# halixness/distributed-3d-diffusion-pytorch

Measured on AMD Instinct MI355X. Metric: train imgs/sec (whole node), SRN cars 64x64 bs128, higher is better.
Workload: dtype bf16; 1 GPU; model=XUNet ch128 ch_mult(1,2,2,4) 136.7M params (3DiM, reference xunet.py), global_batch=128, seq_len=4096, image_size=64, per_gpu_batch=128, micro_batch=128, hip_graph=False, parallelism=dp1, dist_backend=none, tuned_gemms=True, backend=hip

## Files before the change

distributed_3d_diffusion_pytorch_amd/ops/csrc/conv.hip:

```cpp
#include "common.h"
#include <stdlib.h>

#include <algorithm>

D3D_API int d3d_colsum(const float* in, long R, int Cc, float* part, float* out, float* out_odd, int accumulate,
                       hipStream_t st);

typedef __attribute__((ext_vector_type(4))) short s16x4;
typedef __attribute__((ext_vector_type(8))) short s16x8;
typedef __attribute__((address_space(3))) s16x4 lds_s16x4;

namespace {

template <int TAPS, bool TRANS>
__global__ void __launch_bounds__(256, 2)
conv_glds_k(const bf16* __restrict__ I, const bf16* __restrict__ Wp, const float* __restrict__ bias,
            const float* __restrict__ row_bias, const bf16* __restrict__ res, bf16* __restrict__ O,
            const bf16* __restrict__ zero16, int Nimg, int IH, int IW, int IC, int ICp, int OH, int OW, int OC,
            int ldo, int stride, float scale, int res_nmod, float* __restrict__ part, int korder) {
  constexpr int BM = 128, BN = 128, BKk = 64;
  constexpr int WM = 64, WN = 64, TM = 4, TN = 4;
  constexpr int STAGE = (BM + BN) * BKk;
  __shared__ __attribute__((aligned(16))) bf16 smem[2 * STAGE];
  typedef __attribute__((address_space(3))) void lds_void;
// ... 1799 lines not shown
struct WSegs {
  int n;
  int row0[kMaxSegs + 1];
  float* w[kMaxSegs];
  float* b[kMaxSegs];
};

__device__ __forceinline__ int seg_of(const WSegs& sg, int co) {
  int s = 0;
  while (s + 1 < sg.n && co >= sg.row0[s + 1]) ++s;
  return s;
}

__global__ void wgrad_reduce_seg_k(const float* __restrict__ ws, int OC, int IC, int splits, int accumulate,
                                   int taps, const float* __restrict__ bws, int brows, WSegs sg) {
  long total = (long)OC * IC * taps;
  if (bws) {
    for (long c = blockIdx.x * (long)blockDim.x + threadIdx.x; c < OC; c += (long)gridDim.x * blockDim.x) {
      float s = 0.f;
      for (int k = 0; k < brows; ++k) s += bws[(long)k * OC + c];
      int g = seg_of(sg, (int)c);
      float* d = sg.b[g];
      if (d) {
        d += c - sg.row0[g];
        *d = accumulate ? *d + s : s;
      }
    }
  }
  for (long t = blockIdx.x * (long)blockDim.x + threadIdx.x; t < total; t += (long)gridDim.x * blockDim.x) {
    int ci = (int)(t % IC);
    long r = t / IC;
    int tap = (int)(r % taps);
    int co = (int)(r / taps);
    float s0 = 0.f, s1 = 0.f, s2 = 0.f, s3 = 0.f;
    int k = 0;
    for (; k + 4 <= splits; k += 4) {
      s0 += ws[(long)k * total + t];
      s1 += ws[(long)(k + 1) * total + t];
      s2 += ws[(long)(k + 2) * total + t];
      s3 += ws[(long)(k + 3) * total + t];
    }
    for (; k < splits; ++k) s0 += ws[(long)k * total + t];
    float s = (s0 + s1) + (s2 + s3);
    int g = seg_of(sg, co);
    float* d = sg.w[g] + (((long)(co - sg.row0[g]) * IC + ci) * taps + tap);
    *d = accumulate ? *d + s : s;
  }
}

template <int SL>
__global__ void __launch_bounds__(256) wgrad_reduce2_k(const float* __restrict__ ws, int OC, int IC, int taps,
                                                       int splits, int accumulate, const float* __restrict__ bws,
                                                       int brows, float* __restrict__ dW, float* __restrict__ db,
                                                       WSegs sg, int nblk_w, float scale) {
  constexpr int COLS = 256 / SL;
  __shared__ f32x4 red[SL][COLS];
  const int col = threadIdx.x % COLS, sl = threadIdx.x / COLS;
  const bool is_bias = blockIdx.x >= nblk_w;
  const long total = is_bias ? (long)OC : (long)OC * IC * taps;
  const float* src = is_bias ? bws : ws;
  const int nrows = is_bias ? brows : splits;
  const long base = (long)(is_bias ? blockIdx.x - nblk_w : blockIdx.x) * (COLS * 4) + col * 4;
  f32x4 a = {0.f, 0.f, 0.f, 0.f};
  if (base < total) {
    if (base + 3 < total) {
      f32x4 b2 = {0.f, 0.f, 0.f, 0.f};
      int k = sl;
      for (; k + SL < nrows; k += 2 * SL) {
        a += *reinterpret_cast<const f32x4*>(src + (long)k * total + base);
        b2 += *reinterpret_cast<const f32x4*>(src + (long)(k + SL) * total + base);
      }
      if (k < nrows) a += *reinterpret_cast<const f32x4*>(src + (long)k * total + base);
      a += b2;
    } else {
      for (int k = sl; k < nrows; k += SL)
        for (int e = 0; e < 4 && base + e < total; ++e) a[e] += src[(long)k * total + base + e];
    }
  }
  red[sl][col] = a;
  __syncthreads();
  if (sl == 0) {
    f32x4 t = red[0][col];
#pragma unroll
    for (int k = 1; k < SL; ++k) t += red[k][col];
    t *= scale;
    for (int e = 0; e < 4; ++e) {
      const long o = base + e;
      if (o >= total) break;
      float* d;
      if (is_bias) {
        const int c = (int)o;
        if (sg.n > 0) {
          const int g = seg_of(sg, c);
          d = sg.b[g] ? sg.b[g] + (c - sg.row0[g]) : nullptr;
        } else {
          d = db ? db + c : nullptr;
        }
      } else {
        const int ci = (int)(o % IC);
        const long r = o / IC;
        const int tap = (int)(r % taps);
        const int co = (int)(r / taps);
        if (sg.n > 0) {
          const int g = seg_of(sg, co);
          d = sg.w[g] + (((long)(co - sg.row0[g]) * IC + ci) * taps + tap);
        } else {
          d = dW + (((long)co * IC + ci) * taps + tap);
        }
      }
      if (d) *d = accumulate ? *d + t[e] : t[e];
    }
// ... 433 lines not shown
  if (g_conv_impl != CONV_HALO || IC % HALO_CH || OC % 128 || (W != 32 && W != 64) || in_bytes >= (1L << 31) ||
      w_bytes >= (1L << 31) || IC > 512)
    return 0;
  auto nblk = [&](int bn) { return H % (bn / W) ? 0L : (long)N * (H / (bn / W)) * (OC / 128); };
  if ((W != 32 || g_halo_w32) && nblk(512) >= 256) return 0;
  if (W == 32 && g_halo_w32s && nblk(256) >= 256) {
    *tile = 256;
    return 1;
  }
  return 0;
}

D3D_API int d3d_conv3_gn_ok(int N, int H, int W, int IC, int OC) {
  int t = 0;
  return conv3_gn_shape(N, H, W, IC, OC, &t);
}

D3D_API int d3d_conv3_gn(const void* I, const void* Wp, const float* bias, void* O, int N, int H, int W, int IC,
                         int ICp, int OC, float* gnp, int gn_groups, int* gn_done, const float* gab, hipStream_t st) {
  int tile = 0;
  if (gn_done) *gn_done = 0;
  if (!conv3_gn_shape(N, H, W, IC, OC, &tile) || ICp != (IC + 63) / 64 * 64) return -2;
  if (gnp) {
    const int Cg = gn_groups > 0 && OC % gn_groups == 0 ? OC / gn_groups : 0;
    if (!((Cg == 4 || Cg == 8 || Cg == 16 || Cg == 32) && (H * W) % 64 == 0)) gnp = nullptr;
  }
  const long in_bytes = (long)N * H * W * IC * 2, w_bytes = (long)((OC + 127) / 128 * 128) * 9 * ICp * 2;
  dim3 gh((unsigned)(N * (H / (tile / W))), (unsigned)(OC / 128), 1);
  hipLaunchKernelGGL((conv_halo_k<32, false, 256, false, false, true>), gh, dim3(512), 0, st, (const bf16*)I,
                     (const bf16*)Wp, bias, (const float*)nullptr, (const bf16*)nullptr, (bf16*)O, (int)in_bytes,
                     (int)w_bytes, N, H, IC, ICp, OC, 1.f, 0, gnp, gn_groups, (bf16*)nullptr, gab);
  if (gn_done && gnp) *gn_done = 1;
  return (int)hipGetLastError();
}

static void launch_reduce2(const float* ws, int OC, int IC, int taps, int splits, int accumulate, const float* bws,
                           int brows, float* dW, float* db, WSegs sg, bool want_bias, hipStream_t st,
                           float scale = 1.f) {
  if (taps == 9 && sg.n == 0) {
    const long base = (long)OC * ((IC + 63) / 64);
    const int tg = base >= 1024 ? 9 : (base * 3 >= 1024 ? 3 : 1);
    const int nblk_w = (int)(base * (9 / tg));
    const int nblk_b = want_bias ? (OC + 63) / 64 : 0;
#define R9(TGv) hipLaunchKernelGGL(wgrad_reduce9_k<TGv>, dim3(nblk_w + nblk_b), dim3(256), 0, st, ws, OC, IC, splits, \
                                  accumulate, bws, brows, dW, db, nblk_w, scale)
    if (tg == 9) R9(9); else if (tg == 3) R9(3); else R9(1);
#undef R9
    return;
  }
  int SL = 1;
  while (SL < splits && SL < 16) SL <<= 1;
  const long total = (long)OC * IC * taps;
  const int per = 4 * (256 / SL);
  const int nblk_w = (int)((total + per - 1) / per);
  const int nblk_b = want_bias ? (OC + per - 1) / per : 0;
  dim3 grid(nblk_w + nblk_b);
#define RL(S) hipLaunchKernelGGL(wgrad_reduce2_k<S>, grid, dim3(256), 0, st, ws, OC, IC, taps, splits, accumulate, \
                                 bws, brows, dW, db, sg, nblk_w, scale)
  switch (SL) {
    case 1: RL(1); break;
    case 2: RL(2); break;
    case 4: RL(4); break;
    case 8: RL(8); break;
    default: RL(16); break;
  }
#undef RL
}

static void launch_wgrad(const void* dY, const void* I, float* ws, int N, int IH, int IW, int IC, int OH, int OW,
                         int OC, int stride, int pps, int ncb, float* bws, int lw, int lh, int taps, dim3 grid,
                         hipStream_t st, const void* I2 = nullptr, int C1 = 0) {
  constexpr int BM = 128, BN = 128;
  const long in_elems = (long)N * IH * IW * IC;
  const bool wide_long = taps == 1 && (long)OC * IC >= (4L << 20) && pps > 16384;
  const bool fast = stride == 1 && lw >= 0 && IH == OH && IW == OW && IC % 128 == 0;
  if (g_wgrad_impl >= WGRAD_BUFL && !wide_long && (fast || in_elems * 2 < (1L << 31) - (1L << 20)) &&
      (long)pps * OC * 2 < (1L << 31)) {
    constexpr int PK = 32;
#define WB(TP, F)                                                                                                \
  hipLaunchKernelGGL((conv_wgrad_bufl_k<TP, PK, F>), grid, dim3(256), 0, st, (const bf16*)dY, (const bf16*)I, ws,   \
                     (long)N * IH * IW, N, IH, IW, IC, OH, OW, OC, stride, pps, ncb, bws, lw, lh, (const bf16*)I2, C1)
    if (taps == 9 && IC == 64 && !fast && I2 == nullptr) {
      dim3 gp(5, grid.y, grid.z);
      hipLaunchKernelGGL((conv_wgrad_bufl_k<9, PK, false, true>), gp, dim3(256), 0, st, (const bf16*)dY,
                         (const bf16*)I, ws, (long)N * IH * IW, N, IH, IW, IC, OH, OW, OC, stride, pps, 1, bws, lw, lh,
                         (const bf16*)nullptr, 0);
    } else if (taps == 9) {
      if (fast) WB(9, true); else WB(9, false);
    } else {
      if (fast) WB(1, true); else WB(1, false);
    }
#undef WB
    return;
  }
  if (taps == 9)
    hipLaunchKernelGGL((conv_wgrad_k<BM, BN, 9>), grid, dim3(256), 0, st, (const bf16*)dY, (const bf16*)I, ws, N, IH,
                       IW, IC, OH, OW, OC, stride, pps, ncb, bws, lw, lh);
  else
    hipLaunchKernelGGL((conv_wgrad_k<BM, BN, 1>), grid, dim3(256), 0, st, (const bf16*)dY, (const bf16*)I, ws, N, IH,
                       IW, IC, OH, OW, OC, stride, pps, ncb, bws, lw, lh);
}

D3D_API int d3d_conv_wgrad_plan2(int N, int OH, int OW, int OC, int IC, int taps, int* splits, int* pix_per_split) {
  constexpr int BM = 128, BN = 128;
  long P = (long)N * OH * OW;
  int tiles = (taps == 9 && IC == 64 ? 5 : taps * ((IC + BN - 1) / BN)) * ((OC + BM - 1) / BM);
  static const long target = 1024;
  static const bool ceil_ = false;
  long want = ceil_ ? (target + tiles - 1) / tiles : target / tiles;
  long maxs = (P + 255) / 256;
  if (want > maxs) want = maxs;
// ... 180 lines not shown
```

distributed_3d_diffusion_pytorch_amd/ops/csrc/reduce.hip:

```cpp
#include "common.h"

__global__ void __launch_bounds__(256) colsum_part_k(const float* __restrict__ in, long R, int Cc, int rows_per,
                                                     float* __restrict__ part) {
  __shared__ float red[8][33];
  const int c = blockIdx.x * 32 + (threadIdx.x & 31);
  const int rl = threadIdx.x >> 5;
  const long r0 = (long)blockIdx.y * rows_per;
  long r1 = r0 + rows_per;
  if (r1 > R) r1 = R;
  float s = 0.f;
  if (c < Cc)
    for (long r = r0 + rl; r < r1; r += 8) s += in[r * Cc + c];
  red[rl][threadIdx.x & 31] = s;
  __syncthreads();
  if (rl == 0 && c < Cc) {
#pragma unroll
    for (int k = 1; k < 8; ++k) s += red[k][threadIdx.x & 31];
    part[(long)blockIdx.y * Cc + c] = s;
  }
}

namespace {
__global__ void colsum_final_k(const float* __restrict__ part, int RS, int Cc, float* __restrict__ out,
                               float* __restrict__ out_odd, int accumulate) {
  int c = blockIdx.x * blockDim.x + threadIdx.x;
  if (c >= Cc) return;
  float s = 0.f;
  for (int k = 0; k < RS; ++k) s += part[(long)k * Cc + c];
  float* dst = out;
  int idx = c;
  if (out_odd) {
    dst = (c & 1) ? out_odd : out;
    idx = c >> 1;
  }
  dst[idx] = accumulate ? dst[idx] + s : s;
}
}

D3D_API int d3d_colsum(const float* in, long R, int Cc, float* part, float* out, float* out_odd, int accumulate,
                       hipStream_t st) {
  int RS = (int)((R + 63) / 64);
  if (RS > 64) RS = 64;
  if (RS < 1) RS = 1;
  int rows_per = (int)((R + RS - 1) / RS);
  hipLaunchKernelGGL(colsum_part_k, dim3((Cc + 31) / 32, RS), dim3(256), 0, st, in, R, Cc, rows_per, part);
  hipLaunchKernelGGL(colsum_final_k, dim3((Cc + 255) / 256), dim3(256), 0, st, part, RS, Cc, out, out_odd,
                     accumulate);
  return (int)hipGetLastError();
}

struct ColJob {
  const float* in;
  float* out0;
  float* out1;
  int R, Cc, acc, blk0;
};
constexpr int kMaxColJobs = 16;
struct ColJobs {
  ColJob j[kMaxColJobs];
  int n;
};

namespace {
__global__ void __launch_bounds__(256) colsum_jobs_k(ColJobs t) {
  int k = 0;
#pragma unroll 1
  while (k + 1 < t.n && (int)blockIdx.x >= t.j[k + 1].blk0) ++k;
  const ColJob& J = t.j[k];
  const int c = ((int)blockIdx.x - J.blk0) * 256 + (int)threadIdx.x;
  if (c >= J.Cc) return;
  const float* p = J.in + c;
  const long ld = J.Cc;
  float s = 0.f;
  int r = 0;
  for (; r + 8 <= J.R; r += 8) {
    float v[8];
#pragma unroll
    for (int u = 0; u < 8; ++u) v[u] = p[(long)(r + u) * ld];
#pragma unroll
    for (int u = 0; u < 8; ++u) s += v[u];
  }
  for (; r < J.R; ++r) s += p[(long)r * ld];
  float* dst = (c & 1) ? J.out1 : J.out0;
  const int idx = c >> 1;
  dst[idx] = J.acc ? dst[idx] + s : s;
}
}

D3D_API int d3d_colsum_jobs(const ColJob* jobs, int njobs, hipStream_t st) {
  if (njobs < 1 || njobs > kMaxColJobs) return (int)hipErrorInvalidValue;
  ColJobs t{};
  t.n = njobs;
  int blk = 0;
  for (int i = 0; i < njobs; ++i) {
    t.j[i] = jobs[i];
    if (t.j[i].Cc % 2 || t.j[i].R < 1 || !t.j[i].in || !t.j[i].out0 || !t.j[i].out1) return (int)hipErrorInvalidValue;
    t.j[i].blk0 = blk;
    blk += (t.j[i].Cc + 255) / 256;
  }
  hipLaunchKernelGGL(colsum_jobs_k, dim3(blk), dim3(256), 0, st, t);
  return (int)hipGetLastError();
}
```

distributed_3d_diffusion_pytorch_amd/ops/csrc/small_gemm.hip:

```cpp
#include "common.h"

namespace {
constexpr int SG_T = 64, SG_K = 16;
}

__global__ void __launch_bounds__(256) sgemm_strided_k(const float* __restrict__ A, const float* __restrict__ B,
                                                       float* __restrict__ C, int M, int N, int K, long sab, long sam,
                                                       long sak, long sbb, long sbk, long sbn, long scb, long scm,
                                                       long scn, float alpha, float beta) {
  __shared__ float As[SG_K][SG_T + 1];
  __shared__ float Bs[SG_K][SG_T + 1];
  const int b = blockIdx.z;
  const int m0 = blockIdx.y * SG_T, n0 = blockIdx.x * SG_T;
  const int tx = threadIdx.x & 15, ty = threadIdx.x >> 4;
  const float* a = A + (long)b * sab;
  const float* bb = B + (long)b * sbb;
  float acc[4][4] = {};
  for (int k0 = 0; k0 < K; k0 += SG_K) {
    for (int e = threadIdx.x; e < SG_K * SG_T; e += 256) {
      const int kk = e / SG_T, mm = e % SG_T;
      const int gm = m0 + mm, gk = k0 + kk;
      As[kk][mm] = (gm < M && gk < K) ? a[gm * sam + gk * sak] : 0.f;
      const int gn = n0 + mm;
      Bs[kk][mm] = (gn < N && gk < K) ? bb[gk * sbk + gn * sbn] : 0.f;
    }
    __syncthreads();
#pragma unroll
    for (int kk = 0; kk < SG_K; ++kk) {
      float av[4], bv[4];
#pragma unroll
      for (int i = 0; i < 4; ++i) av[i] = As[kk][ty + 16 * i];
#pragma unroll
      for (int j = 0; j < 4; ++j) bv[j] = Bs[kk][tx + 16 * j];
#pragma unroll
      for (int i = 0; i < 4; ++i)
#pragma unroll
        for (int j = 0; j < 4; ++j) acc[i][j] = __builtin_fmaf(av[i], bv[j], acc[i][j]);
    }
    __syncthreads();
  }
  float* c = C + (long)b * scb;
#pragma unroll
  for (int i = 0; i < 4; ++i) {
    const int gm = m0 + ty + 16 * i;
    if (gm >= M) continue;
#pragma unroll
    for (int j = 0; j < 4; ++j) {
      const int gn = n0 + tx + 16 * j;
      if (gn >= N) continue;
      float* d = c + gm * scm + gn * scn;
      *d = beta == 0.f ? alpha * acc[i][j] : alpha * acc[i][j] + beta * *d;
    }
  }
}

D3D_API int d3d_sgemm_strided(const float* A, const float* B, float* C, int M, int N, int K, int batch, long sab,
                              long sam, long sak, long sbb, long sbk, long sbn, long scb, long scm, long scn,
                              float alpha, float beta, hipStream_t st) {
  if (M <= 0 || N <= 0 || K <= 0 || batch <= 0 || batch > 65535) return -1;
  dim3 grid(cdiv(N, SG_T), cdiv(M, SG_T), batch);
  if (grid.y > 65535) return -1;
  hipLaunchKernelGGL(sgemm_strided_k, grid, dim3(256), 0, st, A, B, C, M, N, K, sab, sam, sak, sbb, sbk, sbn, scb,
                     scm, scn, alpha, beta);
  return (int)hipGetLastError();
}

struct SgJob {
  const float* A;
  const float* B;
  float* C;
  bf16* Cb;
  bf16* CbT;
  const float* u;
  const float* v;
  long sam, sak, sbk, sbn, scm, scn;
  int M, N, K, ldb, ldbt, tile0;
  float alpha, beta;
};
static_assert(sizeof(SgJob) == 136, "SgJob must match hip_impl._SgJob");

constexpr int SJ_K = 32;

__global__ void __launch_bounds__(256) sgemm_jobs_k(const SgJob* __restrict__ jobs, int njobs) {
  __shared__ float As[SJ_K][SG_T + 1];
  __shared__ float Bs[SJ_K][SG_T + 1];
  int j = 0;
  while (j + 1 < njobs && (int)blockIdx.x >= jobs[j + 1].tile0) ++j;
  const SgJob& J = jobs[j];
  const int t = blockIdx.x - J.tile0;
  const int ntn = (J.N + SG_T - 1) / SG_T;
  const int m0 = (t / ntn) * SG_T, n0 = (t % ntn) * SG_T;
  const int tx = threadIdx.x & 15, ty = threadIdx.x >> 4;
  float acc[4][4] = {};
  const bool a_k = J.sak == 1, b_k = J.sbk == 1;
  if (J.A) {
    for (int k0 = 0; k0 < J.K; k0 += SJ_K) {
      for (int e = threadIdx.x; e < SJ_K * SG_T; e += 256) {
        int kk = e / SG_T, mm = e % SG_T;
        if (a_k) { kk = e % SJ_K; mm = e / SJ_K; }
        const int gm = m0 + mm, gk = k0 + kk;
        As[kk][mm] = (gm < J.M && gk < J.K) ? J.A[gm * J.sam + gk * J.sak] : 0.f;
        int kb = e / SG_T, nn = e % SG_T;
        if (b_k) { kb = e % SJ_K; nn = e / SJ_K; }
        const int gn = n0 + nn, gkb = k0 + kb;
        Bs[kb][nn] = (gn < J.N && gkb < J.K) ? J.B[gkb * J.sbk + gn * J.sbn] : 0.f;
      }
      __syncthreads();
#pragma unroll 8
      for (int kk = 0; kk < SJ_K; ++kk) {
        float av[4], bv[4];
#pragma unroll
        for (int i = 0; i < 4; ++i) av[i] = As[kk][ty + 16 * i];
#pragma unroll
        for (int q = 0; q < 4; ++q) bv[q] = Bs[kk][tx + 16 * q];
#pragma unroll
        for (int i = 0; i < 4; ++i)
#pragma unroll
          for (int q = 0; q < 4; ++q) acc[i][q] = __builtin_fmaf(av[i], bv[q], acc[i][q]);
      }
      __syncthreads();
    }
  }
#pragma unroll
  for (int i = 0; i < 4; ++i) {
    const int gm = m0 + ty + 16 * i;
    if (gm >= J.M) continue;
    const float um = J.u ? J.u[gm] : 0.f;
#pragma unroll
    for (int q = 0; q < 4; ++q) {
      const int gn = n0 + tx + 16 * q;
      if (gn >= J.N) continue;
      float r = J.alpha * acc[i][q];
      if (J.C && J.beta != 0.f) r += J.beta * J.C[gm * J.scm + gn * J.scn];
      if (J.u) r += um * (J.v ? J.v[gn] : 1.f);
      if (J.C) J.C[gm * J.scm + gn * J.scn] = r;
      if (J.Cb) J.Cb[(long)gm * J.ldb + gn] = (bf16)r;
      if (J.CbT) J.CbT[(long)gn * J.ldbt + gm] = (bf16)r;
    }
  }
}

D3D_API int d3d_sgemm_jobs(const void* jobs, int njobs, int tiles, hipStream_t st) {
  if (njobs <= 0 || tiles <= 0) return -1;
  hipLaunchKernelGGL(sgemm_jobs_k, dim3((unsigned)tiles), dim3(256), 0, st, (const SgJob*)jobs, njobs);
  return (int)hipGetLastError();
}
```

distributed_3d_diffusion_pytorch_amd/ops/csrc/wgrad_group.hip:

```cpp
#include "common.h"

#include <algorithm>

namespace {

typedef __attribute__((ext_vector_type(4))) short gs16x4;
typedef __attribute__((ext_vector_type(8))) short gs16x8;
typedef __attribute__((address_space(3))) gs16x4 glds_s16x4;

__device__ __forceinline__ gs16x4 gw_tr(const bf16* p) {
  return __builtin_amdgcn_ds_read_tr16_b64_v4i16((glds_s16x4*)(p));
}

__device__ __forceinline__ gs16x4 gw_tr_asm(const bf16* p) {
  gs16x4 v;
  const unsigned a = (unsigned)(uintptr_t)(const __attribute__((address_space(3))) void*)p;
  asm volatile("ds_read_b64_tr_b16 %0, %1" : "=v"(v) : "v"(a) : "memory");
  return v;
}
template <int TM, int TN>
__device__ __forceinline__ void gw_tr_wait(bf16x8 (&a)[TM], bf16x8 (&b)[TN]) {
  asm volatile("s_waitcnt lgkmcnt(0)" ::: "memory");
#pragma unroll
  for (int i = 0; i < TM; ++i) asm volatile("" : "+v"(a[i]));
#pragma unroll
  for (int j = 0; j < TN; ++j) asm volatile("" : "+v"(b[j]));
}
__device__ __forceinline__ float gw_dot2(unsigned a, unsigned b, float c) {
  return __builtin_amdgcn_fdot2_f32_bf16(__builtin_bit_cast(bf16x2, a), __builtin_bit_cast(bf16x2, b), c, false);
}

__device__ __forceinline__ __amdgpu_buffer_rsrc_t gw_rsrc(const void* p, long bytes) {
  const unsigned long long a = (unsigned long long)p;
  const unsigned lo = __builtin_amdgcn_readfirstlane((unsigned)a);
  const unsigned hi = __builtin_amdgcn_readfirstlane((unsigned)(a >> 32));
  const int n = __builtin_amdgcn_readfirstlane((int)(bytes > 0 ? (bytes < 0x7fffffffL ? bytes : 0x7fffffffL) : 0));
  return __builtin_amdgcn_make_buffer_rsrc((void*)(((unsigned long long)hi << 32) | lo), (short)0, n, 0x00020000);
}

constexpr int GW_MAX = 16;
constexpr int GW_BM = 128, GW_BN = 128;

struct GwJob {
  const bf16* dy;
  const bf16* x;
  const bf16* x2;
  float* dw;
  float* db;
  float* slab;
  float* bslab;
  long P;
  int OC, IC, C1, taps, H, W, lw, lh, ncb, nmb, splits, pps, blk0, acc;
  float scale;
  int pad_;
};
struct GwTable {
  int n, pad_;
  GwJob j[GW_MAX];
};

struct GrJob {
  const float* slab;
  const float* bslab;
  float* dw;
  float* db;
  int OC, IC, taps, splits, blk0, nblk_w, acc;
  float scale;
  int flat, pad_;
};
struct GrTable {
  int n, pad_;
  GrJob j[GW_MAX];
};

template <int PK>
__device__ __forceinline__ void gw_issue(bf16* sA, bf16* sB, const bf16* __restrict__ dY, const bf16* __restrict__ I,
                                         long in_elems, long p0, long p_end, int OC, int IC, int OH, int OW, int kh,
                                         int kw, int dpix, int lw, int wave, const int* trow, const unsigned* aoff,
                                         const unsigned* boff, const bool* bok, bool on = true) {
  typedef __attribute__((address_space(3))) void lds_void;
  constexpr int PPW = PK / 16;
  const __amdgpu_buffer_rsrc_t rA = gw_rsrc(dY + p0 * OC, on ? (p_end - p0) * OC * 2 : 0);
#pragma unroll
  for (int i = 0; i < PPW; ++i)
    __builtin_amdgcn_raw_ptr_buffer_load_lds(rA, (lds_void*)(sA + (wave * PPW + i) * 4 * GW_BM), 16, aoff[i], 0, 0,
                                             0);
  const long pb = p0 + dpix;
  const __amdgpu_buffer_rsrc_t rB = gw_rsrc(I + pb * IC, on ? (in_elems - pb * IC) * 2 : 0);
  const int wedge = kw == 0 ? 0 : OW - 1, hedge = kh == 0 ? 0 : OH - 1;
#pragma unroll
  for (int i = 0; i < PPW; ++i) {
    const int pp = (int)p0 + trow[i];
    bool bad = !bok[i];
    if (kw != 1) bad |= (pp & (OW - 1)) == wedge;
    if (kh != 1) bad |= ((pp >> lw) & (OH - 1)) == hedge;
    __builtin_amdgcn_raw_ptr_buffer_load_lds(rB, (lds_void*)(sB + (wave * PPW + i) * 4 * GW_BN), 16,
                                             bad ? 0x80000000u : boff[i], 0, 0, 0);
  }
}

}

template <int PK, int NS>
__global__ void __launch_bounds__(256, 2) wgrad_grp_k(GwTable tab) {
  constexpr int BM = GW_BM, BN = GW_BN;
  constexpr int PER = 2 * (PK / 16);
  constexpr int WM = 64, WN = 64, TM = 4, TN = 4;
  constexpr int STAGE = PK * (BM + BN);
  constexpr int PPW = PK / 16;
  __shared__ __attribute__((aligned(16))) bf16 smem[NS * STAGE];
  const int tid = threadIdx.x, lane = tid & 63;
  const int wave = __builtin_amdgcn_readfirstlane(tid >> 6);
  const int wm = wave >> 1, wn = wave & 1;
  int R;
  {
    const int T = gridDim.x, L = blockIdx.x;
    const int q = T / 8, r = T % 8, xcd = L % 8;
    R = (xcd < r ? xcd * (q + 1) : r * (q + 1) + (xcd - r) * q) + L / 8;
  }
  int k = 0;
  while (k + 1 < tab.n && R >= tab.j[k + 1].blk0) ++k;
// ... 373 lines not shown

  const int fr = lane & 15, fq = lane >> 4;
  const int cig = ci0g + 16 * wn + fr;
  const int cw = m0 + 64 * wm;
  if (bias_wave) {
#pragma unroll
    for (int i = 0; i < 4; ++i) {
      bsum[i] += __shfl_xor(bsum[i], 16);
      bsum[i] += __shfl_xor(bsum[i], 32);
    }
  }
  if (splits == 1) {
    const float sc = J.scale;
    const int acc_in = J.acc;
    if (bias_wave && fq == 0) {
#pragma unroll
      for (int i = 0; i < 4; ++i) {
        float* d = J.db + cw + i * 16 + fr;
        const float v = bsum[i] * sc;
        *d = acc_in ? *d + v : v;
      }
    }
#pragma unroll
    for (int i = 0; i < 4; ++i)
#pragma unroll
      for (int e = 0; e < 4; ++e) {
        float* d = J.dw + ((long)(cw + i * 16 + fq * 4 + e) * ICt + cig) * 9;
#pragma unroll
        for (int t = 0; t < 9; ++t) {
          const float v = acc[i][t][e] * sc;
          d[t] = acc_in ? d[t] + v : v;
        }
      }
    return;
  }
  if (bias_wave && fq == 0) {
#pragma unroll
    for (int i = 0; i < 4; ++i) {
      J.bslab[((long)split * 2) * OC + cw + i * 16 + fr] = bsum[i];
      J.bslab[((long)split * 2 + 1) * OC + cw + i * 16 + fr] = 0.f;
    }
  }
  float* slab = J.slab + (long)split * OC * 9L * ICt;
#pragma unroll
  for (int i = 0; i < 4; ++i)
#pragma unroll
    for (int e = 0; e < 4; ++e) {
      float* d = slab + ((long)(cw + i * 16 + fq * 4 + e) * ICt + cig) * 9;
#pragma unroll
      for (int t = 0; t < 9; ++t) d[t] = acc[i][t][e];
    }
}

__global__ void __launch_bounds__(256) wgrad_grp_reduce_k(GrTable tab) {
  __shared__ float red[4][9][64];
  __shared__ float tile[64 * 9];
  const int tid = threadIdx.x;
  const int R = blockIdx.x;
  int k = 0;
  while (k + 1 < tab.n && R >= tab.j[k + 1].blk0) ++k;
  const GrJob& J = tab.j[k];
  const int b = R - J.blk0;
  const int OC = J.OC, IC = J.IC, taps = J.taps, splits = J.splits;
  const int ln = tid >> 6, c = tid & 63;
  if (b >= J.nblk_w) {
    const int co = (b - J.nblk_w) * 64 + c;
    float a0 = 0.f, a1 = 0.f;
    if (co < OC) {
      int r = ln;
      for (; r + 4 < 2 * splits; r += 8) {
        a0 += J.bslab[(long)r * OC + co];
        a1 += J.bslab[(long)(r + 4) * OC + co];
      }
      if (r < 2 * splits) a0 += J.bslab[(long)r * OC + co];
    }
    red[ln][0][c] = a0 + a1;
    __syncthreads();
    if (ln == 0 && co < OC) {
      const float v = (((red[0][0][c] + red[1][0][c]) + red[2][0][c]) + red[3][0][c]) * J.scale;
      J.db[co] = J.acc ? J.db[co] + v : v;
    }
    return;
  }
  if (J.flat) {
    const long total = (long)OC * IC * taps;
    const long e0 = (long)b * 1024 + tid * 4;
    if (e0 >= total) return;
    f32x4 a = *reinterpret_cast<const f32x4*>(J.slab + e0);
    for (int sp = 1; sp < splits; ++sp) a += *reinterpret_cast<const f32x4*>(J.slab + (long)sp * total + e0);
    a *= J.scale;
    f32x4* d = reinterpret_cast<f32x4*>(J.dw + e0);
    *d = J.acc ? *d + a : a;
    return;
  }
  const int ncg = (IC + 63) / 64;
  const int co = b / ncg, ci0 = (b % ncg) * 64;
  const int nci = min(64, IC - ci0);
  const long total = (long)OC * taps * IC;
  float a[9];
#pragma unroll
  for (int t = 0; t < 9; ++t) a[t] = 0.f;
  if (c < nci) {
    const float* src = J.slab + (long)co * taps * IC + ci0 + c;
    for (int sp = ln; sp < splits; sp += 4) {
      const float* s = src + (long)sp * total;
#pragma unroll
      for (int t = 0; t < 9; ++t)
        if (t < taps) a[t] += s[(long)t * IC];
    }
  }
#pragma unroll
  for (int t = 0; t < 9; ++t)
    if (t < taps) red[ln][t][c] = a[t];
  __syncthreads();
  for (int m = tid; m < taps * 64; m += 256) {
    const int t = m >> 6, cc = m & 63;
    tile[cc * taps + t] = (((red[0][t][cc] + red[1][t][cc]) + red[2][t][cc]) + red[3][t][cc]) * J.scale;
  }
  __syncthreads();
  float* dst = J.dw + ((long)co * IC + ci0) * taps;
  for (int m = tid; m < nci * taps; m += 256) dst[m] = J.acc ? dst[m] + tile[m] : tile[m];
}

struct WgJobDesc {
  const void* dy;
  const void* x;
  const void* x2;
  float* dw;
  float* db;
  int N, H, W, OC, IC, C1, taps, acc;
  float scale;
  int pad_;
};
static_assert(sizeof(WgJobDesc) == 80, "WgJobDesc must match hip_impl._WgJob");

static int g_gw_blocks = 512;
static int g_gw_pk = 32;
static int g_gw_minpix = 512;
static int g_gw_ns = 2;
static int g_gh_on = 1;
static int g_gh_blocks = 256;
static int g_gh_blocks_big = 128;
static int g_gh_big_lg2 = 21;
static int g_gh_ns = 2;
static int g_gh_pk = 64;

D3D_API int d3d_wgrad_group_cfg(int blocks, int pk, int minpix) {
  if (blocks > 0) g_gw_blocks = blocks;
  if (pk == 32 || pk == 64) g_gw_pk = pk;
  if (minpix > 0) g_gw_minpix = minpix;
  return 0;
}
D3D_API int d3d_wgrad_group_stages(int ns) {
  if (ns >= 2 && ns <= 4) g_gw_ns = ns;
  return 0;
}
D3D_API int d3d_wgrad_group_halo(int on, int blocks, int ns) {
  if (on >= 0) g_gh_on = on ? 1 : 0;
  if (blocks > 0) g_gh_blocks = blocks;
  if (ns == 2 || ns == 3) g_gh_ns = ns;
  return 0;
}
D3D_API int d3d_wgrad_group_halo_big(int blocks, int lg2) {
  if (blocks > 0) g_gh_blocks_big = blocks;
  if (lg2 > 0) g_gh_big_lg2 = lg2;
  return 0;
}
D3D_API int d3d_wgrad_group_halo_pk(int pk) {
  if (pk == 32 || pk == 64) g_gh_pk = pk;
  return 0;
// ... 124 lines not shown
  if (S.on) gw_plan(S.od, S.on, S.op, false);
  S.ws_floats = S.hp.ws_floats + S.qp.ws_floats + S.op.ws_floats;
}

static long gw_tables(const WgJobDesc* d, int n, const GwPlan& pl, float* ws, bool halo, GwTable& tab, GrTable& rt,
                      long& rblk) {
  tab = GwTable{};
  tab.n = n;
  long blk = 0;
  for (int i = 0; i < n; ++i) {
    GwJob& J = tab.j[i];
    const WgJobDesc& D = d[i];
    J.dy = (const bf16*)D.dy;
    J.x = (const bf16*)D.x;
    J.x2 = (const bf16*)D.x2;
    J.dw = D.dw;
    J.db = D.db;
    J.P = (long)D.N * D.H * D.W;
    J.OC = D.OC;
    J.IC = D.IC;
    J.C1 = D.x2 ? D.C1 : D.IC;
    J.taps = D.taps;
    if (D.taps == 1) {
      J.H = J.W = 1;
      J.lw = J.lh = 0;
    } else {
      J.H = D.H;
      J.W = D.W;
      J.lw = gw_lg2(D.W);
      J.lh = gw_lg2(D.H);
    }
    J.ncb = halo ? D.IC / GH_BN : cdiv(D.IC, GW_BN);
    J.nmb = halo ? D.OC / GH_BM : cdiv(D.OC, GW_BM);
    J.splits = pl.splits[i];
    J.pps = pl.pps[i];
    J.blk0 = (int)blk;
    J.acc = D.acc;
    J.scale = D.scale;
    J.slab = pl.splits[i] > 1 ? ws + pl.slab_off[i] : nullptr;
    J.bslab = pl.splits[i] > 1 && D.db ? ws + pl.bslab_off[i] : nullptr;
    blk += (long)pl.tiles[i] * pl.splits[i];
    if (pl.splits[i] > 1) {
      GrJob& Rj = rt.j[rt.n++];
      Rj.slab = J.slab;
      Rj.bslab = J.bslab;
      Rj.dw = D.dw;
      Rj.db = D.db;
      Rj.OC = D.OC;
      Rj.IC = D.IC;
      Rj.taps = D.taps;
      Rj.splits = pl.splits[i];
      Rj.blk0 = (int)rblk;
      Rj.flat = (halo || D.taps == 1) && ((long)D.OC * D.IC * D.taps) % 4 == 0 && ((uintptr_t)D.dw & 15) == 0;
      Rj.nblk_w = Rj.flat ? (int)cdiv((long)D.OC * D.IC * D.taps, 1024L) : D.OC * cdiv(D.IC, 64);
      Rj.acc = D.acc;
      Rj.scale = D.scale;
      rblk += Rj.nblk_w + (D.db ? cdiv(D.OC, 64) : 0);
    }
  }
  return blk;
}

D3D_API long d3d_wgrad_group(const WgJobDesc* d, int n, float* ws, long ws_floats, hipStream_t st) {
  if (n < 1 || n > GW_MAX) return -1;
  for (int i = 0; i < n; ++i)
    if (d3d_wgrad_group_ok(d + i)) return -2;
  GwSplit S;
  gw_split_plan(d, n, S);
  if (!ws) return S.ws_floats;
  if (ws_floats < S.ws_floats || S.hp.blocks >= (1L << 31) || S.qp.blocks >= (1L << 31) ||
      S.op.blocks >= (1L << 31))
    return -3;
  GrTable rt{};
  long rblk = 0;
  if (S.qn) {
    GwTable tab;
    const long blk = gw_tables(S.qd, S.qn, S.qp, ws + S.hp.ws_floats, true, tab, rt, rblk);
    hipLaunchKernelGGL((wgrad_halo_k<2, 64>), dim3((unsigned)blk), dim3(512), 0, st, tab);
  }
  if (S.hn) {
    GwTable tab;
    const long blk = gw_tables(S.hd, S.hn, S.hp, ws, true, tab, rt, rblk);
    if (g_gh_ns == 3)
      hipLaunchKernelGGL((wgrad_halo_k<3, 32>), dim3((unsigned)blk), dim3(512), 0, st, tab);
    else
      hipLaunchKernelGGL((wgrad_halo_k<2, 32>), dim3((unsigned)blk), dim3(512), 0, st, tab);
  }
  if (S.on) {
    GwTable tab;
    const long blk = gw_tables(S.od, S.on, S.op, ws + S.hp.ws_floats + S.qp.ws_floats, false, tab, rt, rblk);
    if (g_gw_pk == 64) {
      hipLaunchKernelGGL((wgrad_grp_k<64, 2>), dim3((unsigned)blk), dim3(256), 0, st, tab);
    } else if (g_gw_ns == 4) {
      hipLaunchKernelGGL((wgrad_grp_k<32, 4>), dim3((unsigned)blk), dim3(256), 0, st, tab);
    } else if (g_gw_ns == 3) {
      hipLaunchKernelGGL((wgrad_grp_k<32, 3>), dim3((unsigned)blk), dim3(256), 0, st, tab);
    } else {
      hipLaunchKernelGGL((wgrad_grp_k<32, 2>), dim3((unsigned)blk), dim3(256), 0, st, tab);
    }
  }
  if (rt.n > 0) hipLaunchKernelGGL(wgrad_grp_reduce_k, dim3((unsigned)rblk), dim3(256), 0, st, rt);
  const int e = (int)hipGetLastError();
  return e ? -1000 - e : 0;
}

D3D_API int d3d_wgrad_group_plan(const WgJobDesc* d, int n, int* splits, int* pps, long* blocks) {
  if (n < 1 || n > GW_MAX) return -1;
// ... 19 lines not shown
```

Measured before the change: 1136 examples/s.

## Batch loads and shrink tiles in wgrad reduce, colsum and small GEMM kernels

Rewrites several reduction and small-GEMM kernels so that each thread issues a batch of independent loads before accumulating, with sched barriers to keep the loads grouped. Work granularity is also made adaptive, using smaller tiles or chunks when the grid would otherwise have fewer blocks than about twice the CU count. The goal is to raise memory-level parallelism and GPU occupancy for the small, latency-bound kernels in the backward pass. This adds template variants and more complex indexing, and summation order changes slightly.

Result: no change. 1146 examples/s (median of 6 runs) (+0.9%).

```diff
diff --git a/distributed_3d_diffusion_pytorch_amd/ops/csrc/conv.hip b/distributed_3d_diffusion_pytorch_amd/ops/csrc/conv.hip
--- a/distributed_3d_diffusion_pytorch_amd/ops/csrc/conv.hip
+++ b/distributed_3d_diffusion_pytorch_amd/ops/csrc/conv.hip
@@ -1875,11 +1875,72 @@
 __global__ void __launch_bounds__(256) wgrad_reduce2_k(const float* __restrict__ ws, int OC, int IC, int taps,
                                                        int splits, int accumulate, const float* __restrict__ bws,
                                                        int brows, float* __restrict__ dW, float* __restrict__ db,
-                                                       WSegs sg, int nblk_w, float scale) {
+                                                       WSegs sg, int nblk_w, float scale, int wide) {
   constexpr int COLS = 256 / SL;
   __shared__ f32x4 red[SL][COLS];
   const int col = threadIdx.x % COLS, sl = threadIdx.x / COLS;
   const bool is_bias = blockIdx.x >= nblk_w;
+  if (wide > 0 && !is_bias) {
+#pragma clang fp contract(off)
+    if ((int)threadIdx.x * 4 >= wide) return;
+    const long total = (long)OC * IC * taps;
+    const long base = (long)blockIdx.x * wide + threadIdx.x * 4;
+    if (base >= total) return;
+    const bool full = base + 3 < total;
+    const f32x4 z = {0.f, 0.f, 0.f, 0.f};
+    f32x4 v[SL];
+#pragma unroll
+    for (int k = 0; k < SL; ++k) {
+      v[k] = z;
+      if (k < splits) {
+        if (full) {
+          v[k] = *reinterpret_cast<const f32x4*>(ws + (long)k * total + base);
+        } else {
+          for (int e = 0; e < 4 && base + e < total; ++e) v[k][e] = ws[(long)k * total + base + e];
+        }
+      }
+    }
+    __builtin_amdgcn_sched_barrier(0);
+    f32x4 t = z + v[0];
+#pragma unroll
+    for (int k = 1; k < SL; ++k)
+      if (k < splits) t += z + v[k];
+    t *= scale;
+    const long r = base / IC;
+    const int ci = (int)(base - r * IC);
+    if (full && taps == 1 && ci + 3 < IC) {
+      const int co = (int)r;
+      float* d;
+      if (sg.n > 0) {
+        const int g = seg_of(sg, co);
+        d = sg.w[g] + ((long)(co - sg.row0[g]) * IC + ci);
+      } else {
+        d = dW + base;
+      }
+      if (((uintptr_t)d & 15) == 0) {
+        f32x4* d4 = reinterpret_cast<f32x4*>(d);
+        *d4 = accumulate ? *d4 + t : t;
+        return;
+      }
+    }
+    for (int e = 0; e < 4; ++e) {
+      const long o = base + e;
+      if (o >= total) break;
+      const int ce = (int)(o % IC);
+      const long re = o / IC;
+      const int tap = (int)(re % taps);
+      const int co = (int)(re / taps);
+      float* d;
+      if (sg.n > 0) {
+        const int g = seg_of(sg, co);
+        d = sg.w[g] + (((long)(co - sg.row0[g]) * IC + ce) * taps + tap);
+      } else {
+        d = dW + (((long)co * IC + ce) * taps + tap);
+      }
+      *d = accumulate ? *d + t[e] : t[e];
+    }
+    return;
+  }
   const long total = is_bias ? (long)OC : (long)OC * IC * taps;
   const float* src = is_bias ? bws : ws;
   const int nrows = is_bias ? brows : splits;
@@ -2419,11 +2480,17 @@
   while (SL < splits && SL < 16) SL <<= 1;
   const long total = (long)OC * IC * taps;
   const int per = 4 * (256 / SL);
-  const int nblk_w = (int)((total + per - 1) / per);
+  int wide = 0;
+  if (splits <= SL) {
+    wide = 1024;
+    while (wide > 256 && (total + wide - 1) / wide < 2L * device_cus()) wide >>= 1;
+  }
+  const int perw = wide ? wide : per;
+  const int nblk_w = (int)((total + perw - 1) / perw);
   const int nblk_b = want_bias ? (OC + per - 1) / per : 0;
   dim3 grid(nblk_w + nblk_b);
 #define RL(S) hipLaunchKernelGGL(wgrad_reduce2_k<S>, grid, dim3(256), 0, st, ws, OC, IC, taps, splits, accumulate, \
-                                 bws, brows, dW, db, sg, nblk_w, scale)
+                                 bws, brows, dW, db, sg, nblk_w, scale, wide)
   switch (SL) {
     case 1: RL(1); break;
     case 2: RL(2); break;
diff --git a/distributed_3d_diffusion_pytorch_amd/ops/csrc/reduce.hip b/distributed_3d_diffusion_pytorch_amd/ops/csrc/reduce.hip
--- a/distributed_3d_diffusion_pytorch_amd/ops/csrc/reduce.hip
+++ b/distributed_3d_diffusion_pytorch_amd/ops/csrc/reduce.hip
@@ -62,25 +62,44 @@
 };
 
 namespace {
-__global__ void __launch_bounds__(256) colsum_jobs_k(ColJobs t) {
+constexpr int kColBlk = 64;
+
+template <int U>
+__device__ __forceinline__ void colsum_batch(float& s, const float* __restrict__ p, long ld) {
+  float v[U];
+#pragma unroll
+  for (int u = 0; u < U; ++u) v[u] = p[u * ld];
+  __builtin_amdgcn_sched_barrier(0);
+#pragma unroll
+  for (int u = 0; u < U; ++u) s += v[u];
+}
+
+__global__ void __launch_bounds__(kColBlk) colsum_jobs_k(ColJobs t) {
   int k = 0;
 #pragma unroll 1
   while (k + 1 < t.n && (int)blockIdx.x >= t.j[k + 1].blk0) ++k;
   const ColJob& J = t.j[k];
-  const int c = ((int)blockIdx.x - J.blk0) * 256 + (int)threadIdx.x;
+  const int c = ((int)blockIdx.x - J.blk0) * kColBlk + (int)threadIdx.x;
   if (c >= J.Cc) return;
   const float* p = J.in + c;
   const long ld = J.Cc;
+  const int R = J.R;
   float s = 0.f;
   int r = 0;
-  for (; r + 8 <= J.R; r += 8) {
-    float v[8];
-#pragma unroll
-    for (int u = 0; u < 8; ++u) v[u] = p[(long)(r + u) * ld];
-#pragma unroll
-    for (int u = 0; u < 8; ++u) s += v[u];
+  for (; r + 32 <= R; r += 32) colsum_batch<32>(s, p + r * ld, ld);
+  if (r + 16 <= R) {
+    colsum_batch<16>(s, p + r * ld, ld);
+    r += 16;
   }
-  for (; r < J.R; ++r) s += p[(long)r * ld];
+  if (r + 8 <= R) {
+    colsum_batch<8>(s, p + r * ld, ld);
+    r += 8;
+  }
+  if (r + 4 <= R) {
+    colsum_batch<4>(s, p + r * ld, ld);
+    r += 4;
+  }
+  for (; r < R; ++r) s += p[r * ld];
   float* dst = (c & 1) ? J.out1 : J.out0;
   const int idx = c >> 1;
   dst[idx] = J.acc ? dst[idx] + s : s;
@@ -96,8 +115,8 @@
     t.j[i] = jobs[i];
     if (t.j[i].Cc % 2 || t.j[i].R < 1 || !t.j[i].in || !t.j[i].out0 || !t.j[i].out1) return (int)hipErrorInvalidValue;
     t.j[i].blk0 = blk;
-    blk += (t.j[i].Cc + 255) / 256;
+    blk += (t.j[i].Cc + kColBlk - 1) / kColBlk;
   }
-  hipLaunchKernelGGL(colsum_jobs_k, dim3(blk), dim3(256), 0, st, t);
+  hipLaunchKernelGGL(colsum_jobs_k, dim3(blk), dim3(kColBlk), 0, st, t);
   return (int)hipGetLastError();
 }
diff --git a/distributed_3d_diffusion_pytorch_amd/ops/csrc/small_gemm.hip b/distributed_3d_diffusion_pytorch_amd/ops/csrc/small_gemm.hip
--- a/distributed_3d_diffusion_pytorch_amd/ops/csrc/small_gemm.hip
+++ b/distributed_3d_diffusion_pytorch_amd/ops/csrc/small_gemm.hip
@@ -4,48 +4,65 @@
 constexpr int SG_T = 64, SG_K = 16;
 }
 
+template <int T>
 __global__ void __launch_bounds__(256) sgemm_strided_k(const float* __restrict__ A, const float* __restrict__ B,
                                                        float* __restrict__ C, int M, int N, int K, long sab, long sam,
                                                        long sak, long sbb, long sbk, long sbn, long scb, long scm,
                                                        long scn, float alpha, float beta) {
-  __shared__ float As[SG_K][SG_T + 1];
-  __shared__ float Bs[SG_K][SG_T + 1];
+  constexpr int NI = T / 16;
+  constexpr int NL = SG_K * T / 256;
+  __shared__ float As[SG_K][T + 1];
+  __shared__ float Bs[SG_K][T + 1];
   const int b = blockIdx.z;
-  const int m0 = blockIdx.y * SG_T, n0 = blockIdx.x * SG_T;
+  const int m0 = blockIdx.y * T, n0 = blockIdx.x * T;
   const int tx = threadIdx.x & 15, ty = threadIdx.x >> 4;
   const float* a = A + (long)b * sab;
   const float* bb = B + (long)b * sbb;
-  float acc[4][4] = {};
+  const bool a_k = sak < sam, b_k = sbk < sbn;
+  float acc[NI][NI] = {};
   for (int k0 = 0; k0 < K; k0 += SG_K) {
-    for (int e = threadIdx.x; e < SG_K * SG_T; e += 256) {
-      const int kk = e / SG_T, mm = e % SG_T;
-      const int gm = m0 + mm, gk = k0 + kk;
-      As[kk][mm] = (gm < M && gk < K) ? a[gm * sam + gk * sak] : 0.f;
-      const int gn = n0 + mm;
-      Bs[kk][mm] = (gn < N && gk < K) ? bb[gk * sbk + gn * sbn] : 0.f;
+    float ra[NL], rb[NL];
+#pragma unroll
+    for (int l = 0; l < NL; ++l) {
+      const int e = threadIdx.x + l * 256;
+      const int kk = a_k ? e % SG_K : e / T, mm = a_k ? e / SG_K : e % T;
+      const bool ok = m0 + mm < M && k0 + kk < K;
+      ra[l] = a[ok ? (m0 + mm) * sam + (k0 + kk) * sak : 0];
+      const int kb = b_k ? e % SG_K : e / T, nn = b_k ? e / SG_K : e % T;
+      const bool okb = n0 + nn < N && k0 + kb < K;
+      rb[l] = bb[okb ? (k0 + kb) * sbk + (n0 + nn) * sbn : 0];
+    }
+    __builtin_amdgcn_sched_barrier(0);
+#pragma unroll
+    for (int l = 0; l < NL; ++l) {
+      const int e = threadIdx.x + l * 256;
+      const int kk = a_k ? e % SG_K : e / T, mm = a_k ? e / SG_K : e % T;
+      As[kk][mm] = (m0 + mm < M && k0 + kk < K) ? ra[l] : 0.f;
+      const int kb = b_k ? e % SG_K : e / T, nn = b_k ? e / SG_K : e % T;
+      Bs[kb][nn] = (n0 + nn < N && k0 + kb < K) ? rb[l] : 0.f;
     }
     __syncthreads();
 #pragma unroll
     for (int kk = 0; kk < SG_K; ++kk) {
-      float av[4], bv[4];
+      float av[NI], bv[NI];
 #pragma unroll
-      for (int i = 0; i < 4; ++i) av[i] = As[kk][ty + 16 * i];
+      for (int i = 0; i < NI; ++i) av[i] = As[kk][ty + 16 * i];
 #pragma unroll
-      for (int j = 0; j < 4; ++j) bv[j] = Bs[kk][tx + 16 * j];
+      for (int j = 0; j < NI; ++j) bv[j] = Bs[kk][tx + 16 * j];
 #pragma unroll
-      for (int i = 0; i < 4; ++i)
+      for (int i = 0; i < NI; ++i)
 #pragma unroll
-        for (int j = 0; j < 4; ++j) acc[i][j] = __builtin_fmaf(av[i], bv[j], acc[i][j]);
+        for (int j = 0; j < NI; ++j) acc[i][j] = __builtin_fmaf(av[i], bv[j], acc[i][j]);
     }
     __syncthreads();
   }
   float* c = C + (long)b * scb;
 #pragma unroll
-  for (int i = 0; i < 4; ++i) {
+  for (int i = 0; i < NI; ++i) {
     const int gm = m0 + ty + 16 * i;
     if (gm >= M) continue;
 #pragma unroll
-    for (int j = 0; j < 4; ++j) {
+    for (int j = 0; j < NI; ++j) {
       const int gn = n0 + tx + 16 * j;
       if (gn >= N) continue;
       float* d = c + gm * scm + gn * scn;
@@ -58,10 +75,16 @@
                               long sam, long sak, long sbb, long sbk, long sbn, long scb, long scm, long scn,
                               float alpha, float beta, hipStream_t st) {
   if (M <= 0 || N <= 0 || K <= 0 || batch <= 0 || batch > 65535) return -1;
-  dim3 grid(cdiv(N, SG_T), cdiv(M, SG_T), batch);
+  const bool small = (long)cdiv(N, SG_T) * cdiv(M, SG_T) * batch < 2L * device_cus();
+  const int T = small ? 32 : SG_T;
+  dim3 grid(cdiv(N, T), cdiv(M, T), batch);
   if (grid.y > 65535) return -1;
-  hipLaunchKernelGGL(sgemm_strided_k, grid, dim3(256), 0, st, A, B, C, M, N, K, sab, sam, sak, sbb, sbk, sbn, scb,
-                     scm, scn, alpha, beta);
+  if (small)
+    hipLaunchKernelGGL(sgemm_strided_k<32>, grid, dim3(256), 0, st, A, B, C, M, N, K, sab, sam, sak, sbb, sbk, sbn,
+                       scb, scm, scn, alpha, beta);
+  else
+    hipLaunchKernelGGL(sgemm_strided_k<SG_T>, grid, dim3(256), 0, st, A, B, C, M, N, K, sab, sam, sak, sbb, sbk, sbn,
+                       scb, scm, scn, alpha, beta);
   return (int)hipGetLastError();
 }
 
@@ -81,55 +104,74 @@
 
 constexpr int SJ_K = 32;
 
+template <int T>
 __global__ void __launch_bounds__(256) sgemm_jobs_k(const SgJob* __restrict__ jobs, int njobs) {
-  __shared__ float As[SJ_K][SG_T + 1];
-  __shared__ float Bs[SJ_K][SG_T + 1];
+  constexpr int NI = T / 16, SUB = SG_T / T;
+  constexpr int NL = SJ_K * T / 256;
+  __shared__ float As[SJ_K][T + 1];
+  __shared__ float Bs[SJ_K][T + 1];
+  const int tile = (int)blockIdx.x / (SUB * SUB), sub = (int)blockIdx.x % (SUB * SUB);
   int j = 0;
-  while (j + 1 < njobs && (int)blockIdx.x >= jobs[j + 1].tile0) ++j;
+  while (j + 1 < njobs && tile >= jobs[j + 1].tile0) ++j;
   const SgJob& J = jobs[j];
-  const int t = blockIdx.x - J.tile0;
-  const int ntn = (J.N + SG_T - 1) / SG_T;
-  const int m0 = (t / ntn) * SG_T, n0 = (t % ntn) * SG_T;
+  const int t = tile - J.tile0;
+  const int M = J.M, N = J.N, K = J.K;
+  const int ntn = (N + SG_T - 1) / SG_T;
+  const int m0 = (t / ntn) * SG_T + (sub / SUB) * T, n0 = (t % ntn) * SG_T + (sub % SUB) * T;
+  if (m0 >= M || n0 >= N) return;
   const int tx = threadIdx.x & 15, ty = threadIdx.x >> 4;
-  float acc[4][4] = {};
-  const bool a_k = J.sak == 1, b_k = J.sbk == 1;
-  if (J.A) {
-    for (int k0 = 0; k0 < J.K; k0 += SJ_K) {
-      for (int e = threadIdx.x; e < SJ_K * SG_T; e += 256) {
-        int kk = e / SG_T, mm = e % SG_T;
-        if (a_k) { kk = e % SJ_K; mm = e / SJ_K; }
-        const int gm = m0 + mm, gk = k0 + kk;
-        As[kk][mm] = (gm < J.M && gk < J.K) ? J.A[gm * J.sam + gk * J.sak] : 0.f;
-        int kb = e / SG_T, nn = e % SG_T;
-        if (b_k) { kb = e % SJ_K; nn = e / SJ_K; }
-        const int gn = n0 + nn, gkb = k0 + kb;
-        Bs[kb][nn] = (gn < J.N && gkb < J.K) ? J.B[gkb * J.sbk + gn * J.sbn] : 0.f;
+  float acc[NI][NI] = {};
+  const float* __restrict__ A = J.A;
+  const float* __restrict__ B = J.B;
+  const long sam = J.sam, sak = J.sak, sbk = J.sbk, sbn = J.sbn;
+  const bool a_k = sak == 1, b_k = sbk == 1;
+  if (A) {
+    for (int k0 = 0; k0 < K; k0 += SJ_K) {
+      float ra[NL], rb[NL];
+#pragma unroll
+      for (int l = 0; l < NL; ++l) {
+        const int e = threadIdx.x + l * 256;
+        const int kk = a_k ? e % SJ_K : e / T, mm = a_k ? e / SJ_K : e % T;
+        const bool ok = m0 + mm < M && k0 + kk < K;
+        ra[l] = A[ok ? (m0 + mm) * sam + (k0 + kk) * sak : 0];
+        const int kb = b_k ? e % SJ_K : e / T, nn = b_k ? e / SJ_K : e % T;
+        const bool okb = n0 + nn < N && k0 + kb < K;
+        rb[l] = B[okb ? (k0 + kb) * sbk + (n0 + nn) * sbn : 0];
+      }
+      __builtin_amdgcn_sched_barrier(0);
+#pragma unroll
+      for (int l = 0; l < NL; ++l) {
+        const int e = threadIdx.x + l * 256;
+        const int kk = a_k ? e % SJ_K : e / T, mm = a_k ? e / SJ_K : e % T;
+        As[kk][mm] = (m0 + mm < M && k0 + kk < K) ? ra[l] : 0.f;
+        const int kb = b_k ? e % SJ_K : e / T, nn = b_k ? e / SJ_K : e % T;
+        Bs[kb][nn] = (n0 + nn < N && k0 + kb < K) ? rb[l] : 0.f;
       }
       __syncthreads();
 #pragma unroll 8
       for (int kk = 0; kk < SJ_K; ++kk) {
-        float av[4], bv[4];
+        float av[NI], bv[NI];
 #pragma unroll
-        for (int i = 0; i < 4; ++i) av[i] = As[kk][ty + 16 * i];
+        for (int i = 0; i < NI; ++i) av[i] = As[kk][ty + 16 * i];
 #pragma unroll
-        for (int q = 0; q < 4; ++q) bv[q] = Bs[kk][tx + 16 * q];
+        for (int q = 0; q < NI; ++q) bv[q] = Bs[kk][tx + 16 * q];
 #pragma unroll
-        for (int i = 0; i < 4; ++i)
+        for (int i = 0; i < NI; ++i)
 #pragma unroll
-          for (int q = 0; q < 4; ++q) acc[i][q] = __builtin_fmaf(av[i], bv[q], acc[i][q]);
+          for (int q = 0; q < NI; ++q) acc[i][q] = __builtin_fmaf(av[i], bv[q], acc[i][q]);
       }
       __syncthreads();
     }
   }
 #pragma unroll
-  for (int i = 0; i < 4; ++i) {
+  for (int i = 0; i < NI; ++i) {
     const int gm = m0 + ty + 16 * i;
-    if (gm >= J.M) continue;
+    if (gm >= M) continue;
     const float um = J.u ? J.u[gm] : 0.f;
 #pragma unroll
-    for (int q = 0; q < 4; ++q) {
+    for (int q = 0; q < NI; ++q) {
       const int gn = n0 + tx + 16 * q;
-      if (gn >= J.N) continue;
+      if (gn >= N) continue;
       float r = J.alpha * acc[i][q];
       if (J.C && J.beta != 0.f) r += J.beta * J.C[gm * J.scm + gn * J.scn];
       if (J.u) r += um * (J.v ? J.v[gn] : 1.f);
@@ -142,6 +184,9 @@
 
 D3D_API int d3d_sgemm_jobs(const void* jobs, int njobs, int tiles, hipStream_t st) {
   if (njobs <= 0 || tiles <= 0) return -1;
-  hipLaunchKernelGGL(sgemm_jobs_k, dim3((unsigned)tiles), dim3(256), 0, st, (const SgJob*)jobs, njobs);
+  if (tiles < 2 * device_cus())
+    hipLaunchKernelGGL(sgemm_jobs_k<32>, dim3((unsigned)tiles * 4), dim3(256), 0, st, (const SgJob*)jobs, njobs);
+  else
+    hipLaunchKernelGGL(sgemm_jobs_k<SG_T>, dim3((unsigned)tiles), dim3(256), 0, st, (const SgJob*)jobs, njobs);
   return (int)hipGetLastError();
 }
diff --git a/distributed_3d_diffusion_pytorch_amd/ops/csrc/wgrad_group.hip b/distributed_3d_diffusion_pytorch_amd/ops/csrc/wgrad_group.hip
--- a/distributed_3d_diffusion_pytorch_amd/ops/csrc/wgrad_group.hip
+++ b/distributed_3d_diffusion_pytorch_amd/ops/csrc/wgrad_group.hip
@@ -66,7 +66,7 @@
   float* db;
   int OC, IC, taps, splits, blk0, nblk_w, acc;
   float scale;
-  int flat, pad_;
+  int flat, gran;
 };
 struct GrTable {
   int n, pad_;
@@ -546,8 +546,37 @@
     }
 }
 
+typedef __attribute__((address_space(1))) const f32x4 gr_gf32x4;
+__device__ __forceinline__ f32x4 gr_load4(const float* p, unsigned off) {
+  const unsigned long long a = (unsigned long long)p;
+  const unsigned lo = __builtin_amdgcn_readfirstlane((unsigned)a);
+  const unsigned hi = __builtin_amdgcn_readfirstlane((unsigned)(a >> 32));
+  const unsigned long long u = ((unsigned long long)hi << 32) | lo;
+  return *(gr_gf32x4*)(u + (unsigned long long)off * 4);
+}
+
+constexpr int GR_FLAT_U = 8;
+template <int U>
+__device__ __forceinline__ void gr_flat_batch(f32x4& a, const float* __restrict__ p, long stride, unsigned off) {
+  f32x4 v[U];
+#pragma unroll
+  for (int u = 0; u < U; ++u) v[u] = gr_load4(p + u * stride, off);
+  __builtin_amdgcn_sched_barrier(0);
+#pragma unroll
+  for (int u = 0; u < U; ++u) a += v[u];
+}
+template <int U>
+__device__ __forceinline__ void gr_tap_batch(f32x4 (&r)[4], const float* __restrict__ p, long stride, unsigned off) {
+  f32x4 v[U];
+#pragma unroll
+  for (int u = 0; u < U; ++u) v[u] = gr_load4(p + u * stride, off);
+  __builtin_amdgcn_sched_barrier(0);
+#pragma unroll
+  for (int u = 0; u < U; ++u) r[u & 3] += v[u];
+}
+
 __global__ void __launch_bounds__(256) wgrad_grp_reduce_k(GrTable tab) {
-  __shared__ float red[4][9][64];
+  __shared__ float red[4][64];
   __shared__ float tile[64 * 9];
   const int tid = threadIdx.x;
   const int R = blockIdx.x;
@@ -556,60 +585,92 @@
   const GrJob& J = tab.j[k];
   const int b = R - J.blk0;
   const int OC = J.OC, IC = J.IC, taps = J.taps, splits = J.splits;
-  const int ln = tid >> 6, c = tid & 63;
   if (b >= J.nblk_w) {
+    const int ln = tid >> 6, c = tid & 63;
     const int co = (b - J.nblk_w) * 64 + c;
     float a0 = 0.f, a1 = 0.f;
     if (co < OC) {
+      const float* p = J.bslab + co;
+      const int rows = 2 * splits;
       int r = ln;
-      for (; r + 4 < 2 * splits; r += 8) {
-        a0 += J.bslab[(long)r * OC + co];
-        a1 += J.bslab[(long)(r + 4) * OC + co];
-      }
-      if (r < 2 * splits) a0 += J.bslab[(long)r * OC + co];
-    }
-    red[ln][0][c] = a0 + a1;
+      for (; r + 28 < rows; r += 32) {
+        float v[8];
+#pragma unroll
+        for (int u = 0; u < 8; ++u) v[u] = p[(long)(r + 4 * u) * OC];
+        __builtin_amdgcn_sched_barrier(0);
+#pragma unroll
+        for (int u = 0; u < 8; u += 2) {
+          a0 += v[u];
+          a1 += v[u + 1];
+        }
+      }
+      for (; r + 4 < rows; r += 8) {
+        const float v0 = p[(long)r * OC], v1 = p[(long)(r + 4) * OC];
+        a0 += v0;
+        a1 += v1;
+      }
+      if (r < rows) a0 += p[(long)r * OC];
+    }
+    red[ln][c] = a0 + a1;
     __syncthreads();
     if (ln == 0 && co < OC) {
-      const float v = (((red[0][0][c] + red[1][0][c]) + red[2][0][c]) + red[3][0][c]) * J.scale;
+      const float v = (((red[0][c] + red[1][c]) + red[2][c]) + red[3][c]) * J.scale;
       J.db[co] = J.acc ? J.db[co] + v : v;
     }
     return;
   }
+  const long total = (long)OC * IC * taps;
   if (J.flat) {
-    const long total = (long)OC * IC * taps;
-    const long e0 = (long)b * 1024 + tid * 4;
+    if (tid * 4 >= J.gran) return;
+    const long e0 = (long)b * J.gran + tid * 4;
     if (e0 >= total) return;
-    f32x4 a = *reinterpret_cast<const f32x4*>(J.slab + e0);
-    for (int sp = 1; sp < splits; ++sp) a += *reinterpret_cast<const f32x4*>(J.slab + (long)sp * total + e0);
+    const float* p = J.slab + (long)b * J.gran;
+    const unsigned off = tid * 4;
+    f32x4 a = {-0.f, -0.f, -0.f, -0.f};
+    int sp = 0;
+    for (; sp + GR_FLAT_U <= splits; sp += GR_FLAT_U) gr_flat_batch<GR_FLAT_U>(a, p + sp * total, total, off);
+    if (sp + 4 <= splits) {
+      gr_flat_batch<4>(a, p + sp * total, total, off);
+      sp += 4;
+    }
+    if (sp + 2 <= splits) {
+      gr_flat_batch<2>(a, p + sp * total, total, off);
+      sp += 2;
+    }
+    if (sp < splits) gr_flat_batch<1>(a, p + sp * total, total, off);
     a *= J.scale;
     f32x4* d = reinterpret_cast<f32x4*>(J.dw + e0);
     *d = J.acc ? *d + a : a;
     return;
   }
-  const int ncg = (IC + 63) / 64;
-  const int co = b / ncg, ci0 = (b % ncg) * 64;
-  const int nci = min(64, IC - ci0);
-  const long total = (long)OC * taps * IC;
-  float a[9];
-#pragma unroll
-  for (int t = 0; t < 9; ++t) a[t] = 0.f;
-  if (c < nci) {
-    const float* src = J.slab + (long)co * taps * IC + ci0 + c;
-    for (int sp = ln; sp < splits; sp += 4) {
-      const float* s = src + (long)sp * total;
-#pragma unroll
-      for (int t = 0; t < 9; ++t)
-        if (t < taps) a[t] += s[(long)t * IC];
-    }
-  }
-#pragma unroll
-  for (int t = 0; t < 9; ++t)
-    if (t < taps) red[ln][t][c] = a[t];
-  __syncthreads();
-  for (int m = tid; m < taps * 64; m += 256) {
-    const int t = m >> 6, cc = m & 63;
-    tile[cc * taps + t] = (((red[0][t][cc] + red[1][t][cc]) + red[2][t][cc]) + red[3][t][cc]) * J.scale;
+  const int cw = J.gran, qw = cw >> 2;
+  const int ncg = (IC + cw - 1) / cw;
+  const int co = b / ncg, ci0 = (b % ncg) * cw;
+  const int nci = min(cw, IC - ci0);
+  const int t = tid / qw, q = tid % qw;
+  if (t < taps && 4 * q < nci) {
+    const float* src = J.slab + (long)co * taps * IC + ci0;
+    const unsigned off = t * IC + 4 * q;
+    f32x4 r[4];
+#pragma unroll
+    for (int i = 0; i < 4; ++i) r[i] = f32x4{0.f, 0.f, 0.f, 0.f};
+    int sp = 0;
+    for (; sp + 8 <= splits; sp += 8) gr_tap_batch<8>(r, src + sp * total, total, off);
+    if (sp + 4 <= splits) {
+      gr_tap_batch<4>(r, src + sp * total, total, off);
+      sp += 4;
+    }
+    if (sp + 2 <= splits) {
+      gr_tap_batch<2>(r, src + sp * total, total, off);
+      sp += 2;
+    }
+    if (sp < splits) {
+      const f32x4 v = gr_load4(src + sp * total, off);
+      if (sp & 2) r[2] += v; else r[0] += v;
+    }
+    const f32x4 s = (((r[0] + r[1]) + r[2]) + r[3]) * J.scale;
+#pragma unroll
+    for (int e = 0; e < 4; ++e) tile[(4 * q + e) * taps + t] = s[e];
   }
   __syncthreads();
   float* dst = J.dw + ((long)co * IC + ci0) * taps;
@@ -840,7 +901,16 @@
       Rj.splits = pl.splits[i];
       Rj.blk0 = (int)rblk;
       Rj.flat = (halo || D.taps == 1) && ((long)D.OC * D.IC * D.taps) % 4 == 0 && ((uintptr_t)D.dw & 15) == 0;
-      Rj.nblk_w = Rj.flat ? (int)cdiv((long)D.OC * D.IC * D.taps, 1024L) : D.OC * cdiv(D.IC, 64);
+      const long want = 2L * device_cus(), tot = (long)D.OC * D.IC * D.taps;
+      if (Rj.flat) {
+        Rj.gran = 1024;
+        while (Rj.gran > 256 && cdiv(tot, (long)Rj.gran) < want) Rj.gran >>= 1;
+        Rj.nblk_w = (int)cdiv(tot, (long)Rj.gran);
+      } else {
+        Rj.gran = 64;
+        while (Rj.gran > 16 && (long)D.OC * cdiv(D.IC, Rj.gran) < want) Rj.gran >>= 1;
+        Rj.nblk_w = D.OC * cdiv(D.IC, Rj.gran);
+      }
       Rj.acc = D.acc;
       Rj.scale = D.scale;
       rblk += Rj.nblk_w + (D.db ? cdiv(D.OC, 64) : 0);
```
